# kehanxuuu/vspg-pbrt-v4

Measured on AMD Instinct MI355X. Metric: Mpaths/sec on 1920x1080 homogeneous fog; relMSE vs CPU ref at equal spp, higher is better.
Workload: dtype f32; 1 GPU; fog-box 1920x1080, guidedvolpathvspg vspguiding=true (primary-ray VSP; App. F options), 1 spp per step per GPU, independent sampler seed 0, maxdepth 5

## Files before the change

vspg-pbrt-v4_amd/csrc/vspg_capi.hip:

```cpp
#include <hip/hip_runtime.h>
#include <dlfcn.h>

#include <cmath>
#include <cstdio>
#include <cstdlib>
#include <cstring>
#include <string>
#include <type_traits>
#include <vector>
#include <algorithm>

#include "vspg_path.h"
#include "vspg_wg_kernel.h"
#include "vspg_guided_wg.h"
#include "vspg_wg3.h"
#include "vspg_trace.h"
#include "vspg_wavefront.h"
#include "vspg_wf_launch.h"
#include "vspg_film_error.h"
#ifdef VSPG_SINGLE_TU
#include "vspg_wf_grid.hip"
#include "vspg_wf_nvdb.hip"
#include "vspg_wg3_exact.hip"
#endif
// ... 1494 lines not shown
    float *le_scale = nullptr;
    float *temperature = nullptr;
    float *majorant = nullptr;
    DTri *tris = nullptr;
    DBvh4Node *bvh = nullptr;
    float *wf_pool = nullptr;
    float4 *wave_samples[2] = {nullptr, nullptr};
    int ws_cur = 0;
    bool ws_parked = false;
    PixelWindow ws_win = {0, 0, 0, 0};
    hipStream_t ws_stream = nullptr;
    hipEvent_t ws_event = nullptr;
    unsigned int *carry_img[2] = {nullptr, nullptr};
    int carry_cur = 0;
    bool carry_pending = false;
    Wg3Launch carry_shape = {};
    int carry_arith = 0;
    unsigned long long carry_resumes = 0;
    unsigned int *wf_lists = nullptr;
    hipStream_t wf_stream2 = nullptr;
    hipEvent_t wf_ev_vertex = nullptr, wf_ev_shadow = nullptr;
    WfIter *wf_iters = nullptr;
    size_t wf_items = 0;
    int num_cus = 0;
    int vsp_ready = 0;
    bool vsp_loaded = false;
    int wave_counter = 0, buffer_wave = 0;
    size_t npix = 0;
    float4 *fe_ref = nullptr;
    bool fe_ref_set = false;
// ... 1388 lines not shown
static bool wg2_defer_enabled() {
    const char *e = getenv("VSPG_WG2_DEFER");
    return !(e && e[0] == '0');
}
static int order_after_parking(VspgRenderer *r, hipStream_t s) {
    if (r->ws_parked && r->ws_event && s != r->ws_stream) HIPCHK(hipStreamWaitEvent(s, r->ws_event, 0));
    return 0;
}
static bool wg3_carry_enabled() {
    const char *e = getenv("VSPG_WG3_CARRY");
    return !(e && e[0] == '0') && wg2_defer_enabled();
}
static int wg3_launch_any(int arith, const Wg3Launch &L) {
    return arith == VSPG_ARITH_FAST_WEIGHTS ? vspg_arith1_wg3(&L) : arith == VSPG_ARITH_FAST ? vspg_arith2_wg3(&L) : wg3_launch_exact(L);
}
static int drain_carried_paths(VspgRenderer *r, hipStream_t s) {
    if (!r->carry_pending) return 0;
    if (const int rc = order_after_parking(r, s)) return rc;
    Wg3Launch L = r->carry_shape;
    L.vsp_ready = r->vsp_ready;
    L.first_sample = -1;
    L.work_head = r->work_head8 + (r->head8_parity & 1u) * (unsigned)(kWg3HeadSetBytes / 4);
    L.ws_prev = nullptr;
    L.ws_out = r->wave_samples[r->ws_cur ^ 1];
    L.stream = s;
    L.carry = 1;
    L.resume = r->carry_img[r->carry_cur ^ 1];
    L.suspend = nullptr;
    const int lrc = wg3_launch_any(r->carry_arith, L);
    if (lrc != 0) return fail(VSPG_EHIP, std::string("k_render_wave_wg3_carry (drain): ") + hipGetErrorName((hipError_t)lrc));
    r->carry_pending = false;
    r->ws_stream = s;
    if (r->ws_event) HIPCHK(hipEventRecord(r->ws_event, s));
    return 0;
}
static int flush_parked_samples(VspgRenderer *r, hipStream_t s) {
    if (const int rc = drain_carried_paths(r, s)) return rc;
    if (!r->ws_parked) return 0;
    if (const int rc = order_after_parking(r, s)) return rc;
    const size_t n_win = (size_t)(r->ws_win.x1 - r->ws_win.x0) * (size_t)(r->ws_win.y1 - r->ws_win.y0);
    hipLaunchKernelGGL(k_film_resolve, dim3((unsigned)((n_win + kBlock - 1) / kBlock)), dim3(kBlock), 0, s, r->cfg.xres, r->ws_win,
                       r->wave_samples[r->ws_cur ^ 1], r->film, r->isg_stats);
    HIPCHK(hipGetLastError());
    r->ws_parked = false;
    return 0;
}
static const char *kernel_name_exact(VspgRenderer *r);
const char *vspg_renderer_kernel_name(VspgRenderer *r) {
    if (!r) return "";
    if (r->arith == VSPG_ARITH_EXACT) return kernel_name_exact(r);
    r->kernel_name_buf = std::string(r->arith == VSPG_ARITH_FAST_WEIGHTS ? "fastw::" : "fast::") + kernel_name_exact(r);
    return r->kernel_name_buf.c_str();
// ... 89 lines not shown
    const int sc = r->cfg.shard_count, si = r->cfg.shard_index;
    int first = wave_start;
    if (sc > 1) first += ((si - wave_start % sc) % sc + sc) % sc;
    if (first >= wave_end) return 0;
    const int n_samples = (wave_end - 1 - first) / sc + 1;
    const PcgJump jump = pcg_jump((unsigned long long)first * 65536ull);
    const bool grid = r->scene.medium.type == VSPG_MEDIUM_GRID;
    const bool nvdb = r->scene.medium.type == VSPG_MEDIUM_NANOVDB;
    const bool guided = wants_guiding(r->prm);
    if (guided && !r->field_set) return fail(VSPG_ESCOPE, "guiding enabled but the renderer holds no guiding field");
    const bool defer = !uses_wf_pipeline(r) && uses_wg2(r) && n_samples == 1 && wg2_defer_enabled();
    const bool same_win = r->ws_win.x0 == x0 && r->ws_win.y0 == y0 && r->ws_win.x1 == x1 && r->ws_win.y1 == y1;
    if (!defer || !same_win) { const int rc = flush_parked_samples(r, (hipStream_t)stream); if (rc) return rc; }
    const bool carry = defer && uses_wg3(r) && !r->hscene.tr_calc && wg3_carry_enabled();
    if (r->carry_pending && !carry) { const int rc = drain_carried_paths(r, (hipStream_t)stream); if (rc) return rc; }
    if (uses_wf_pipeline(r)) {
#ifdef VSPG_WF_DEBUG
        auto checksum = [&](const void *dptr, size_t bytes) -> unsigned long long {
            if (!dptr || !bytes) return 0ull;
            std::vector<unsigned char> h(bytes);
            (void)hipDeviceSynchronize();
            (void)hipMemcpy(h.data(), dptr, bytes, hipMemcpyDeviceToHost);
            unsigned long long x = 1469598103934665603ull;
            for (size_t i = 0; i < bytes; ++i) { x ^= h[i]; x *= 1099511628211ull; }
            return x;
        };
        const size_t nb = (size_t)r->hscene.bnx * r->hscene.bny * r->hscene.bnz;
        const void *bufs[6] = {r->tris, r->bvh, r->brick_index, r->octets, r->dscene, r->majorant};
        const size_t sizes[6] = {(size_t)r->hscene.n_tris * sizeof(DTri), (size_t)r->hscene.n_bvh_nodes * sizeof(DBvh4Node), nb * 4, r->n_bricks * 512 * 32,
                                 sizeof(DScene), (size_t)16 * 16 * 16 * 4};
// ... 50 lines not shown
        long long wblocks = (long long)r->num_cus * (wwaves * 4 / (wblock / 64));
        const long long wmax = (items + kWgChunk - 1) / kWgChunk;
        if (wblocks > wmax) wblocks = wmax;
        const int single = n_samples == 1 ? 1 : 0;
        const long long n_tiles_all = (long long)tilesX * tilesY;
        const bool sched2 = uses_wg2(r);
        if (sched2) {
            for (int k = 0; k < 2; ++k)
                if (!r->wave_samples[k]) HIPCHK(hipMalloc(&r->wave_samples[k], r->npix * sizeof(float4)));
            const int wg3_grey = r->medium_grey ? (r->surfaces_grey ? 2 : 1) : 0, wg3_null_zero = r->medium_grey && r->surfaces_grey && r->null_zero ? 1 : 0;
            if (carry && wblocks > n_tiles_all) wblocks = n_tiles_all;
            if (r->carry_pending) {
                const Wg3Launch &P = r->carry_shape;
                const bool same_shape = carry && P.grey == wg3_grey && P.null_zero == wg3_null_zero && P.blocks == (unsigned)wblocks && P.windowed == (whole ? 0 : 1) &&
                                        r->carry_arith == r->arith && P.first_sample != first && P.dscene == r->dscene;
                if (!same_shape) { const int rc = drain_carried_paths(r, (hipStream_t)stream); if (rc) return rc; }
            }
            float4 *const ws_out = r->wave_samples[r->ws_cur];
            const float4 *const ws_prev = defer && r->ws_parked ? r->wave_samples[r->ws_cur ^ 1] : nullptr;
            if (ws_prev) { const int rc = order_after_parking(r, (hipStream_t)stream); if (rc) return rc; }
            const long long n_tiles = n_tiles_all;
            if (wblocks > n_tiles) wblocks = n_tiles;
            const int tail64 = [] { const char *e = getenv("VSPG_WG2_TAIL"); const int v = e ? atoi(e) : 64; return v < 0 ? 0 : (v > 64 ? 64 : v); }();
            const unsigned static_tiles = (unsigned)((n_tiles * (64 - tail64) / 64) / wblocks * wblocks);
#define VSPG_LAUNCH_WG2(M, G, NPOOL, BLK, WV)                                                                                         \
    hipLaunchKernelGGL((k_render_wave_wg2<M, G, NPOOL, BLK, WV>), dim3((unsigned)wblocks), dim3(BLK), 0, (hipStream_t)stream, r->dscene, \
                       r->film, r->isg_stats, r->vsp, r->vsp_ready, wave_end, first, single, jump, tiles_magic, static_tiles, work_head, ws_prev, ws_out, r->counters, targs, win)
            if (uses_wg3(r)) {
                {
                    static_assert(kWgBlockHomog == VSPG_WG_BLOCK && kWgWavesHomog == VSPG_WG_WAVES, "wg3_launch_unguided's launch shape");
                    unsigned int *const head8 = r->work_head8 + (r->head8_parity & 1u) * (unsigned)(kWg3HeadSetBytes / 4);
// ... 189 lines not shown
        }
        while (std::pow(2.0, (double)r->buffer_wave) <= (double)r->wave_counter) r->buffer_wave++;
    }
    return 0;
}
int vspg_post_process_wave(VspgRenderer *r, void *stream) { return vspg_post_process_step(r, 1, nullptr, stream); }
int vspg_renderer_set_exchange(VspgRenderer *r, VspgExchangeFn fn, void *user) {
    if (!r) return fail(VSPG_EINVAL, "null renderer");
    r->exchange = fn;
    r->exchange_user = user;
    return 0;
}

int vspg_flush(VspgRenderer *r, void *stream) {
    if (!r) return fail(VSPG_EINVAL, "null renderer");
    if (!r->ws_parked) return 0;
    HIPCHK(hipSetDevice(r->cfg.device));
    return flush_parked_samples(r, (hipStream_t)stream);
}
long long vspg_debug_carry_resumes(VspgRenderer *r) { return r ? (long long)r->carry_resumes : -1; }
int vspg_film_device_ptr(VspgRenderer *r, float **dev_ptr, size_t *n_floats) {
    if (!r || !dev_ptr || !n_floats) return fail(VSPG_EINVAL, "null argument");
    if (r->ws_parked) {
        HIPCHK(hipSetDevice(r->cfg.device));
        const hipStream_t s = r->ws_stream;
        if (const int rc = flush_parked_samples(r, s)) return rc;
        HIPCHK(hipStreamSynchronize(s));
    }
    *dev_ptr = reinterpret_cast<float *>(r->film);
    *n_floats = r->npix * 4;
    return 0;
}
int vspg_film_read(VspgRenderer *r, float *host, void *stream) {
    if (!r || !host) return fail(VSPG_EINVAL, "null argument");
    HIPCHK(hipSetDevice(r->cfg.device));
    if (const int rc = flush_parked_samples(r, (hipStream_t)stream)) return rc;
    HIPCHK(hipMemcpyAsync(host, r->film, r->npix * sizeof(float4), hipMemcpyDeviceToHost, (hipStream_t)stream));
    HIPCHK(hipStreamSynchronize((hipStream_t)stream));
// ... 115 lines not shown
    HIPCHK(hipStreamSynchronize(s));
    return 0;
}
int vspg_vsp_buffer_load(VspgRenderer *r, const float *host, void *stream) {
    if (!r || !host) return fail(VSPG_EINVAL, "null argument");
    HIPCHK(hipSetDevice(r->cfg.device));
    if (const int rc = flush_parked_samples(r, (hipStream_t)stream)) return rc;
    HIPCHK(hipMemcpyAsync(r->vsp, host, r->npix * sizeof(float), hipMemcpyHostToDevice, (hipStream_t)stream));
    HIPCHK(hipStreamSynchronize((hipStream_t)stream));
    r->vsp_ready = 1;
    r->vsp_loaded = true;
    return 0;
}
int vspg_isg_stats_device_ptr(VspgRenderer *r, float **dev_ptr, size_t *n_floats) {
    if (!r || !dev_ptr || !n_floats) return fail(VSPG_EINVAL, "null argument");
    if (r->ws_parked) {
        HIPCHK(hipSetDevice(r->cfg.device));
        const hipStream_t s = r->ws_stream;
        if (const int rc = flush_parked_samples(r, s)) return rc;
        HIPCHK(hipStreamSynchronize(s));
    }
    *dev_ptr = r->isg_stats;
    *n_floats = r->npix * VSPG_ISG_STATS;
    return 0;
}
int vspg_get_counters(VspgRenderer *r, VspgCounters *out, void *stream) {
    if (!r || !out) return fail(VSPG_EINVAL, "null argument");
    HIPCHK(hipSetDevice(r->cfg.device));
    if (const int rc = drain_carried_paths(r, (hipStream_t)stream)) return rc;
    unsigned long long h[kNumCounters];
    HIPCHK(hipMemcpyAsync(h, r->counters, sizeof h, hipMemcpyDeviceToHost, (hipStream_t)stream));
// ... 404 lines not shown
```

vspg-pbrt-v4_amd/csrc/vspg_wg3.h:

```cpp
#pragma once
#include <type_traits>

#include "vspg_guided_wg.h"
#include "vspg_path.h"
#include "vspg_wg_kernel.h"

VSPG_NS_BEGIN

enum { Q_VV = 0, Q_VS = 1, Q_A = 2, Q_F = 3, Q_COUNT = 4 };
enum { QC_RES = 0, QC_COM = 1, QC_HEAD = 2, QC_STRIDE = 4 };
enum { W3_BUSY_S = Q_COUNT * QC_STRIDE, W3_BUSY_V, W3_EXH, W3_LIVE, W3_COUNT };
enum { W3_OLD = Q_VV * QC_STRIDE + 3, W3_SUSP_LO = Q_VS * QC_STRIDE + 3, W3_SUSP_HI = Q_A * QC_STRIDE + 3 };
constexpr unsigned kCarryDrainBit = 0x80000000u;
enum { W3_NONE = 0, W3_VERTEX = 1, W3_SEGMENT = 2, W3_FRESH = 3, W3_EXIT = 4 };
constexpr unsigned kRestartBit = 0x8000u;

VDEV float isg_code(const IsgSample &isg) {
    if (!isg.valid) return 0.f;
    const float q = isg.vsp_used >= 0.f ? isg.vsp_used : 0.5f;
    return isg.surface_event ? -q : q;
}
__device__ __forceinline__ void resolve_sample(float4 s, float4 *film_px, float *isg_px) {
    const Spec L = Spec{s.x, s.y, s.z};
    film_add_sample_rmw(film_px, L);
    IsgSample isg;
    isg.valid = s.w != 0.f;
    isg.surface_event = s.w < 0.f;
    isg.vsp_used = __builtin_fabsf(s.w);
// ... 5 lines not shown
    return v;
}
__device__ __forceinline__ int w3_lane() {
    int l = (int)(threadIdx.x & 63u);
    asm volatile("" : "+v"(l));
    return l;
}
constexpr float kCarrySentinel = 2.f;
__device__ __forceinline__ bool carry_sentinel(float w) { return w > 1.f; }
template <class LY, int NP> constexpr int kWg3ImagePool = LY::COUNT * NP;
template <class LY, int NP> constexpr int kWg3ImageWords = LY::COUNT * NP + Q_COUNT * NP / 2;
template <class LY, int NP> constexpr int kWg3ImageStride = kWg3ImageWords<LY, NP> + 32;
static_assert(W3_COUNT <= 32, "the image's queue words");

constexpr int kWg3Heads = 8, kWg3HeadSetBytes = kWg3Heads * 128;
__device__ __forceinline__ void reset_sibling_head(unsigned int *work_head) {
    if (blockIdx.x == 0 && threadIdx.x == 0) *reinterpret_cast<unsigned int *>(reinterpret_cast<uintptr_t>(work_head) ^ 4u) = 0u;
}

typedef unsigned int w3_u32x4 __attribute__((ext_vector_type(4)));
typedef const volatile __attribute__((address_space(3))) w3_u32x4 *w3_lds_v4;
template <int NP>
VDEV void ring_push_all(int dq, unsigned entry, unsigned short (*ring)[NP], unsigned int *s_w) {
    const int lane = w3_lane();
    const unsigned long long m0 = __ballot(dq == 0), m1 = __ballot(dq == 1), m2 = __ballot(dq == 2), m3 = __ballot(dq == 3);
    const unsigned n0 = (unsigned)__popcll(m0), n1 = (unsigned)__popcll(m1), n2 = (unsigned)__popcll(m2), n3 = (unsigned)__popcll(m3);
    const unsigned myn = lane == 0 ? n0 : lane == 1 ? n1 : lane == 2 ? n2 : n3;
    unsigned base = 0;
    if (lane < Q_COUNT && myn > 0u) base = atomicAdd(s_w + lane * QC_STRIDE + QC_RES, myn);
    const unsigned b0 = (unsigned)__builtin_amdgcn_readlane((int)base, 0), b1 = (unsigned)__builtin_amdgcn_readlane((int)base, 1);
// ... 14 lines not shown
#define VSPG_WG3_NP_CAP 768
#endif
#ifndef VSPG_WG3_LDS_BUDGET
#define VSPG_WG3_LDS_BUDGET 81920
#endif
#ifndef VSPG_WG3_OTHER
#define VSPG_WG3_OTHER 5200
#endif
template <class LY>
constexpr int wg3_pool_paths(int other_bytes) {
    const int n = (VSPG_WG3_LDS_BUDGET - other_bytes) / (LY::COUNT * 4 + Q_COUNT * 2) / 32 * 32;
    return n < VSPG_WG3_NP_CAP ? n : VSPG_WG3_NP_CAP;
}

#ifdef VSPG_W3_TIMELINE
enum { W3T_BEGIN = 0, W3T_FULL, W3T_EXH, W3T_EXIT, W3T_SUMS, W3T_WORDS = W3T_SUMS + 27, W3T_MAX_BLOCKS = 2048 };
__device__ unsigned long long g_w3_timeline[W3T_MAX_BLOCKS][8][32];
struct W3Timeline {
    unsigned long long *rec, t0;
    unsigned phase;
    __device__ __forceinline__ bool mine() const { return (threadIdx.x & 63u) == 0u && blockIdx.x < (unsigned)W3T_MAX_BLOCKS; }
    __device__ __forceinline__ W3Timeline() : rec(&g_w3_timeline[blockIdx.x % W3T_MAX_BLOCKS][(threadIdx.x >> 6) & 7u][0]), t0(0), phase(0) { stamp(W3T_BEGIN); }
    __device__ __forceinline__ void stamp(int i) { const unsigned long long t = __builtin_amdgcn_s_memrealtime(); if (mine()) rec[i] = t; }
    __device__ __forceinline__ void enter(unsigned p, int i) { if (phase < p) { phase = p; stamp(i); } }
    __device__ __forceinline__ void chunk_begin() { t0 = __builtin_amdgcn_s_memrealtime(); }
    __device__ __forceinline__ void chunk_end(unsigned kind, unsigned lanes) {
        const unsigned long long t1 = __builtin_amdgcn_s_memrealtime();
        if (mine()) {
            unsigned long long *r = rec + W3T_SUMS + (phase * 3u + kind) * 3u;
            atomicAdd(r, 1ull); atomicAdd(r + 1, (unsigned long long)lanes); atomicAdd(r + 2, t1 - t0);
        }
    }
};
#define VSPG_W3T(x) x
#else
#define VSPG_W3T(x)
#endif

template <class Medium, bool GUIDED, int NP, int kWgBlock, int kWgWavesPerSimd, bool TRAIN, bool WINDOW, bool CARRY = false>
__device__ __forceinline__ void wg3_render(
    const DScene *__restrict__ Sp, float4 *__restrict__ film, float *__restrict__ isg_stats, const float *__restrict__ vsp_buf,
    int vsp_ready, int wave_end, int first_sample, int single_sample, PcgJump jump, unsigned int tiles_magic,
    unsigned int *__restrict__ work_head, const float4 *__restrict__ prev_samples,
    float4 *__restrict__ wave_samples, unsigned long long *__restrict__ counters, TrainArgs train, const PixelWindow win,
    const unsigned int *__restrict__ resume = nullptr, unsigned int *__restrict__ suspend = nullptr) {
    static_assert(!CARRY || (!TRAIN && !GUIDED), "CARRY serves the unguided one-sample launches");
    vsp_ready = w3_at_use(vsp_ready), wave_end = w3_at_use(wave_end), first_sample = w3_at_use(first_sample);
    single_sample = w3_at_use(single_sample);
    const DScene &S = *Sp;
    const int W = S.xres, H = S.yres;
    const int tilesX = WINDOW ? win_tiles_x(win) : (W + 7) >> 3, tilesY = WINDOW ? win_tiles_y(win) : (H + 7) >> 3;
    const unsigned n_tiles = CARRY && w3_at_use(suspend) == nullptr ? 0u : (unsigned)(tilesX * tilesY);
    const auto in_launch = [&](int px, int py) {
        if constexpr (WINDOW) return win_has(win, px, py);
        else return px < W && py < H;
    };
    const int lane = threadIdx.x & 63;
    const int sample_step = S.shard_count > 1 ? S.shard_count : 1;
    if (blockIdx.x == 0 && threadIdx.x < (unsigned)kWg3Heads)
        reinterpret_cast<unsigned int *>(reinterpret_cast<uintptr_t>(work_head) ^ (uintptr_t)kWg3HeadSetBytes)[threadIdx.x * 32u] = 0u;
    unsigned wseg = blockIdx.x % (unsigned)kWg3Heads, wtried = 0u;

    constexpr bool FULL = !Medium::kSimpleScene;
    static_assert(!FULL || !GUIDED, "the workgroup kernel's guided vertex (vspg_guided_wg.h) is built for rectangle scenes");
    static_assert(NP < (int)kRestartBit, "a ring entry is the slot plus the restart bit");
    using LY = PoolLayout<GUIDED, Medium::kGrey, TRAIN, FULL>;
    constexpr int NF = LY::COUNT;
    static_assert(!TRAIN || GUIDED, "segment recording belongs to the guided instantiations");
    static_assert(Medium::kSingleSegment, "k_render_wave_wg3 serves homogeneous media (grid media: the wavefront pipeline)");
    __shared__ float s_pool[NF * NP];
    __shared__ unsigned short s_ring[Q_COUNT][NP];
    __shared__ __attribute__((aligned(16))) unsigned int s_w[W3_COUNT];
    const Pool P{s_pool, NP};
    const Medium medium = MediumMaker<Medium>::make(S, nullptr);
    float *glds = nullptr;
    if constexpr (GUIDED && kKdLdsNodes > 0) {
        __shared__ VspgKdNode s_kd[2][kKdLdsNodes > 0 ? kKdLdsNodes : 1];
        for (int f = 0; f < 2; ++f) {
            const int nl = S.field[f].n_nodes < kKdLdsNodes ? S.field[f].n_nodes : kKdLdsNodes;
            for (int i = threadIdx.x; i < nl; i += kWgBlock) s_kd[f][i] = S.field[f].nodes[i];
        }
        glds = reinterpret_cast<float *>(&s_kd[0][0]);
    }
    __shared__ unsigned int s_counters[CNT_COUNT];
    struct LaneCounters : PathCounters { uint32_t paths; VDEV void path() { paths++; } };
    using Rec = typename std::conditional<TRAIN, PathRecorder, NullRecorder>::type;
// ... 7 lines not shown
            const unsigned tcol = WINDOW ? (px >> 3) - (unsigned)win_tile_x0(win) : px >> 3, trow = WINDOW ? (py >> 3) - (unsigned)win_tile_y0(win) : py >> 3;
            const unsigned item = (trow * (unsigned)tilesX + tcol) * 64u + ((py & 7u) << 3) + (px & 7u);
            pc.rec.base = train.segbuf + item;
            pc.rec.stride = (int)train.n_items;
            pc.rec.max_seg = train_rec_capacity(S.prm.maxdepth);
            return item;
        } else {
            (void)pxy;
            return 0u;
        }
    };

    stage_scene_lds(S);
    if (threadIdx.x < CNT_COUNT) s_counters[threadIdx.x] = 0;
    constexpr int kImgPool = kWg3ImagePool<LY, NP>, kImgWords = kWg3ImageWords<LY, NP>, kImgStride = kWg3ImageStride<LY, NP>;
    bool resumed = false;
    if constexpr (CARRY) {
        const unsigned int *const img = resume + (size_t)blockIdx.x * kImgStride;
        resumed = resume != nullptr && img[kImgWords + W3_LIVE] != 0u;
        if (resumed) {
            unsigned int *const pool32 = reinterpret_cast<unsigned int *>(s_pool);
#pragma unroll 8
            for (int i = threadIdx.x; i < kImgPool; i += kWgBlock) pool32[i] = img[i];
            unsigned short *const ring16 = &s_ring[0][0];
#pragma unroll 3
            for (int i = threadIdx.x; i < Q_COUNT * NP / 2; i += kWgBlock) {
                const unsigned v = img[kImgPool + i];
                ring16[2 * i] = (unsigned short)(v & 0xffffu);
                ring16[2 * i + 1] = (unsigned short)(v >> 16);
            }
            if (threadIdx.x < W3_COUNT) s_w[threadIdx.x] = img[kImgWords + threadIdx.x];
            __syncthreads();
            if (threadIdx.x < Q_COUNT) {
                const unsigned h = s_w[threadIdx.x * QC_STRIDE + QC_HEAD], n = s_w[threadIdx.x * QC_STRIDE + QC_COM] - h, h2 = h % (unsigned)NP;
                s_w[threadIdx.x * QC_STRIDE + QC_HEAD] = h2;
                s_w[threadIdx.x * QC_STRIDE + QC_RES] = h2 + n;
                s_w[threadIdx.x * QC_STRIDE + QC_COM] = h2 + n;
            }
            if (threadIdx.x == 0) {
                s_w[W3_OLD] = s_w[W3_LIVE];
                s_w[W3_EXH] = 0u;
                s_w[W3_BUSY_S] = 0u;
                s_w[W3_BUSY_V] = 0u;
            }
        }
    }
    if (!resumed) {
        if (threadIdx.x < W3_COUNT) s_w[threadIdx.x] = 0;
        for (int i = threadIdx.x; i < NP; i += kWgBlock) s_ring[Q_F][i] = (unsigned short)i;
        __syncthreads();
        if (threadIdx.x == 0) {
            s_w[Q_F * QC_STRIDE + QC_RES] = NP; s_w[Q_F * QC_STRIDE + QC_COM] = NP;
        }
    }
    if constexpr (CARRY) {
        __syncthreads();
        if (threadIdx.x == 0) {
            if (suspend == nullptr) { s_w[W3_EXH] = 1u; s_w[W3_OLD] |= kCarryDrainBit; }
            s_w[W3_SUSP_LO] = (unsigned)reinterpret_cast<uintptr_t>(suspend);
            s_w[W3_SUSP_HI] = (unsigned)(reinterpret_cast<uintptr_t>(suspend) >> 32);
        }
    }
    __syncthreads();

    auto emit = [&](int pxy, Spec Lraw, const IsgSample &isg, bool old) {
        const Spec L = finish_radiance(Lraw);
        const size_t pidx = (size_t)((unsigned)pxy >> 16) * W + (pxy & 0xffff);
        if (CARRY && old && w3_at_use(first_sample) >= 0) {
            resolve_sample(make_float4(L.r, L.g, L.b, isg_code(isg)), film + pidx, isg_stats + pidx * VSPG_ISG_STATS);
        } else if (w3_at_use(single_sample)) {
            wave_samples[pidx] = make_float4(L.r, L.g, L.b, isg_code(isg));
        } else {
            film_add_sample(film + pidx, L);
            isg_add_sample_atomic(isg_stats + pidx * VSPG_ISG_STATS, L, isg);
        }
    };

    VSPG_PROF(PS_WG_TOTAL);
    VSPG_PROF_ACC(prof_decide, PS_WG_R);
    VSPG_PROF_ACC(prof_idle, PS_WG_BAR_A);
    unsigned idle_polls = 0;
    VSPG_W3T(W3Timeline tl);
    while (true) {
        VSPG_PROF_ACC_BEGIN(prof_decide);
        VSPG_PROF_ACC_BEGIN(prof_idle);
        unsigned kind = W3_NONE, pos0 = 0, n0 = 0, pos1 = 0, n1 = 0, q0 = Q_VV, tile = 0;
        unsigned fresh_entry = 0;
        {
            const auto U = [](unsigned v) { return (unsigned)__builtin_amdgcn_readfirstlane((int)v); };
            const w3_lds_v4 qw = (w3_lds_v4)(s_w);
            const w3_u32x4 wVV = qw[Q_VV], wVS = qw[Q_VS], wA = qw[Q_A], wF = qw[Q_F], wM = qw[Q_COUNT];
            const unsigned hVV = U(wVV.z), hVS = U(wVS.z), hA = U(wA.z), hF = U(wF.z);
            const unsigned busyS = U(wM.x), busyV = U(wM.y), live = U(wM.w);
            const unsigned old_word = CARRY ? U(wVV.w) : 1u;
            const bool exh = U(wM.z) != 0u;
            VSPG_W3T(if (exh) tl.enter(2u, W3T_EXH));
            const auto avail = [&](w3_u32x4 q, unsigned head) {
                const unsigned r = U(q.x), c = U(q.y);
                const int a = (int)(c - head);
                return r == c && a > 0 ? a : 0;
            };
            const int aVV = avail(wVV, hVV), aVS = avail(wVS, hVS), aA = avail(wA, hA), aF = exh ? 0 : avail(wF, hF);
            const auto claim = [&](unsigned q, unsigned head, unsigned n) {
                unsigned old = head + 1u;
                if (w3_lane() == 0) old = atomicCAS(s_w + q * QC_STRIDE + QC_HEAD, head, head + n);
                return U(old) == head;
            };
            const auto bump = [&](int w, int d) { if (w3_lane() == 0) atomicAdd(s_w + w, (unsigned)d); };
            const auto claim_vertex = [&](int a_first, unsigned h_first, unsigned q_first, int a_second, unsigned h_second, unsigned q_second) {
                bump(W3_BUSY_V, 1);
// ... 13 lines not shown
                else bump(W3_BUSY_S, -1);
            };
            const int aV = aVV + aVS;
            if (CARRY && exh && old_word == 0u) kind = W3_EXIT;
            else if (aVV >= 64) claim_vertex(aVV, hVV, Q_VV, 0, hVS, Q_VS);
            else if (aVS >= 64) claim_vertex(aVS, hVS, Q_VS, 0, hVV, Q_VV);
            else if (aA >= 64) claim_segment();
            else if (aF >= 64) {
                bump(W3_BUSY_S, 1);
                bump(W3_LIVE, 64);
                if (claim(Q_F, hF, 64u)) {
                    kind = W3_FRESH; pos0 = hF; n0 = 64u;
                    __builtin_amdgcn_fence(__ATOMIC_ACQUIRE, "workgroup");
                    fresh_entry = s_ring[Q_F][(hF + (unsigned)lane) % (unsigned)NP];
                    tile = n_tiles;
                    while (wtried < (unsigned)kWg3Heads) {
                        unsigned c = 0xffffffffu;
                        if (w3_lane() == 0 && __hip_atomic_load(work_head + wseg * 32u, __ATOMIC_RELAXED, __HIP_MEMORY_SCOPE_AGENT) * (unsigned)kWg3Heads + wseg < n_tiles)
                            c = atomicAdd(work_head + wseg * 32u, 1u);
                        c = U(c);
                        if (c != 0xffffffffu && c * (unsigned)kWg3Heads + wseg < n_tiles) {
                            tile = c * (unsigned)kWg3Heads + wseg;
                            break;
                        }
                        wseg = (wseg + 1u) % (unsigned)kWg3Heads;
                        ++wtried;
                    }
                } else {
                    bump(W3_LIVE, -64);
                    bump(W3_BUSY_S, -1);
                }
            } else if (aV >= 64 || (aV > 0 && busyS == 0u)) {
                if (aVV >= aVS) claim_vertex(aVV, hVV, Q_VV, aVS, hVS, Q_VS);
                else claim_vertex(aVS, hVS, Q_VS, aVV, hVV, Q_VV);
            } else if (aA > 0 && busyV == 0u) {
                claim_segment();
            } else if (exh && live == 0u) {
                kind = W3_EXIT;
            }
        }
        if (kind == W3_EXIT) break;
        if (kind == W3_NONE) {
            if (idle_polls < 2u) __builtin_amdgcn_s_sleep(2);
            else __builtin_amdgcn_s_sleep(VSPG_WG3_IDLE_SLEEP);
            VSPG_PROF_ACC_END(prof_idle);
            if (++idle_polls > (1u << 23)) break;
            continue;
        }
        VSPG_PROF_ACC_END(prof_decide);
        idle_polls = 0;
        VSPG_W3T(if (kind == W3_VERTEX && n0 + n1 == 64u) tl.enter(1u, W3T_FULL); tl.chunk_begin());
        __builtin_amdgcn_fence(__ATOMIC_ACQUIRE, "workgroup");

        if (kind == W3_VERTEX) {
            VSPG_PROF(PS_WG_B);
            bool cont = false, restart = false, freed = false, old_done = false;
            int slot = 0;
            if ((unsigned)lane < n0 + n1) {
                slot = (unsigned)lane < n0 ? s_ring[q0][(pos0 + (unsigned)lane) % (unsigned)NP]
                                           : s_ring[q0 ^ 1u][(pos1 + ((unsigned)lane - n0)) % (unsigned)NP];
// ... 152 lines not shown
    VSPG_W3T(tl.stamp(W3T_EXIT));
    if constexpr (!GUIDED) {
        atomicAdd(&s_counters[CNT_PATHS], pc.paths); atomicAdd(&s_counters[CNT_SEGMENTS], pc.segments);
        atomicAdd(&s_counters[CNT_VOLUME_SCATTERS], pc.volume_scatters); atomicAdd(&s_counters[CNT_SURFACE_HITS], pc.surface_hits);
        atomicAdd(&s_counters[CNT_DENSITY_QUERIES], pc.density_queries); atomicAdd(&s_counters[CNT_SHADOW_RAYS], pc.shadow_rays);
        atomicAdd(&s_counters[CNT_SHADOW_QUERIES], pc.shadow_queries);
    }
    __syncthreads();
    if (threadIdx.x < CNT_COUNT) atomicAdd(&counters[threadIdx.x], (unsigned long long)s_counters[threadIdx.x]);
    if constexpr (CARRY) {
        unsigned int *const susp = reinterpret_cast<unsigned int *>((uintptr_t)s_w[W3_SUSP_LO] | ((uintptr_t)s_w[W3_SUSP_HI] << 32));
        if (susp != nullptr) {
            unsigned int *const img = susp + (size_t)blockIdx.x * kImgStride;
            if (threadIdx.x < W3_COUNT) img[kImgWords + threadIdx.x] = s_w[threadIdx.x];
            if (s_w[W3_LIVE] != 0u) {
                const unsigned int *const pool32 = reinterpret_cast<const unsigned int *>(s_pool);
                for (int i = threadIdx.x; i < kImgPool; i += kWgBlock) img[i] = pool32[i];
                const unsigned short *const ring16 = &s_ring[0][0];
                for (int i = threadIdx.x; i < Q_COUNT * NP / 2; i += kWgBlock) img[kImgPool + i] = (unsigned)ring16[2 * i] | ((unsigned)ring16[2 * i + 1] << 16);
                for (int q = 0; q < Q_F; ++q) {
                    const unsigned h = s_w[q * QC_STRIDE + QC_HEAD], n = s_w[q * QC_STRIDE + QC_COM] - h;
                    for (unsigned i = threadIdx.x; i < n && i < (unsigned)NP; i += kWgBlock) {
                        const int pxy = P.i(LY::PIXEL, (int)(s_ring[q][(h + i) % (unsigned)NP] & (kRestartBit - 1u)) % NP);
                        const unsigned px = (unsigned)pxy & 0xffffu, py = (unsigned)pxy >> 16;
                        if (in_launch((int)px, (int)py)) wave_samples[(size_t)py * W + px].w = kCarrySentinel;
                    }
                }
            }
        }
    }
}

template <class Medium, bool GUIDED, int NP, int kWgBlock, int kWgWavesPerSimd, bool TRAIN = false>
__global__ __launch_bounds__(kWgBlock, kWgWavesPerSimd) void k_render_wave_wg3(
    const DScene *__restrict__ Sp, float4 *__restrict__ film, float *__restrict__ isg_stats, const float *__restrict__ vsp_buf,
    int vsp_ready, int wave_end, int first_sample, int single_sample, PcgJump jump, unsigned int tiles_magic,
    unsigned int *__restrict__ work_head, const float4 *__restrict__ prev_samples,
    float4 *__restrict__ wave_samples, unsigned long long *__restrict__ counters, TrainArgs train = TrainArgs{nullptr, nullptr, nullptr, nullptr, 0, 0}) {
    wg3_render<Medium, GUIDED, NP, kWgBlock, kWgWavesPerSimd, TRAIN, false>(Sp, film, isg_stats, vsp_buf, vsp_ready, wave_end, first_sample, single_sample, jump,
                                                                            tiles_magic, work_head, prev_samples, wave_samples, counters, train, PixelWindow{0, 0, 0, 0});
}
template <class Medium, bool GUIDED, int NP, int kWgBlock, int kWgWavesPerSimd, bool TRAIN = false>
__global__ __launch_bounds__(kWgBlock, kWgWavesPerSimd) void k_render_wave_wg3_window(
    const DScene *__restrict__ Sp, float4 *__restrict__ film, float *__restrict__ isg_stats, const float *__restrict__ vsp_buf,
    int vsp_ready, int wave_end, int first_sample, int single_sample, PcgJump jump, unsigned int tiles_magic,
// ... 82 lines not shown
```

vspg-pbrt-v4_amd/csrc/vspg_wg3_exact.hip:

```cpp
#include <hip/hip_runtime.h>

#include "vspg_wg3.h"

VSPG_NS_BEGIN
int wg3_launch_exact(const Wg3Launch &L) { return wg3_launch_unguided(L); }
VSPG_NS_END

#ifdef VSPG_W3_TIMELINE
extern "C" int vspg_w3_timeline_read(unsigned long long *out, int blocks) {
    using namespace vspg;
    if (blocks < 0 || blocks > (int)W3T_MAX_BLOCKS) return -1;
    const size_t bytes = (size_t)blocks * 8 * 32 * sizeof(unsigned long long);
    if (hipDeviceSynchronize() != hipSuccess) return -2;
    if (hipMemcpyFromSymbol(out, HIP_SYMBOL(g_w3_timeline), bytes) != hipSuccess) return -3;
    void *p = nullptr;
    if (hipGetSymbolAddress(&p, HIP_SYMBOL(g_w3_timeline)) != hipSuccess || hipMemset(p, 0, sizeof(g_w3_timeline)) != hipSuccess) return -4;
    return 0;
}
#endif
```

Measured before the change: 3628 Mpaths/s.

## Fuse carried-path drain with parked-sample resolve and vectorize suspend images

When flushing, the carried-path drain launch now also resolves the parked wave samples and claims fresh tiles (exact arithmetic only), so a separate film-resolve kernel is no longer needed. In the carry kernel, exhaustion is detected by polling the global work heads, and a 'thin' drain mode relaxes the vertex/segment batching thresholds so stragglers finish sooner. The suspend and resume copies of the LDS image now use 128-bit accesses instead of 32-bit and 16-bit ones. Timeline instrumentation is extended with poll and branch counters. The changes add state (drain_behind) and cross-stream ordering that must stay correct for film reads.

```diff
diff --git a/vspg-pbrt-v4_amd/csrc/vspg_capi.hip b/vspg-pbrt-v4_amd/csrc/vspg_capi.hip
--- a/vspg-pbrt-v4_amd/csrc/vspg_capi.hip
+++ b/vspg-pbrt-v4_amd/csrc/vspg_capi.hip
@@ -1532,6 +1532,7 @@
     unsigned int *carry_img[2] = {nullptr, nullptr};
     int carry_cur = 0;
     bool carry_pending = false;
+    bool drain_behind = false;
     Wg3Launch carry_shape = {};
     int carry_arith = 0;
     unsigned long long carry_resumes = 0;
@@ -2950,14 +2951,21 @@
 static int wg3_launch_any(int arith, const Wg3Launch &L) {
     return arith == VSPG_ARITH_FAST_WEIGHTS ? vspg_arith1_wg3(&L) : arith == VSPG_ARITH_FAST ? vspg_arith2_wg3(&L) : wg3_launch_exact(L);
 }
-static int drain_carried_paths(VspgRenderer *r, hipStream_t s) {
+static int drain_carried_paths(VspgRenderer *r, hipStream_t s, bool resolve = false) {
     if (!r->carry_pending) return 0;
     if (const int rc = order_after_parking(r, s)) return rc;
+    resolve = resolve && r->ws_parked && r->carry_arith == VSPG_ARITH_EXACT;
     Wg3Launch L = r->carry_shape;
     L.vsp_ready = r->vsp_ready;
-    L.first_sample = -1;
     L.work_head = r->work_head8 + (r->head8_parity & 1u) * (unsigned)(kWg3HeadSetBytes / 4);
-    L.ws_prev = nullptr;
+    if (resolve) {
+        L.first_sample = L.wave_end = kCarryDrainResolve;
+        r->head8_parity ^= 1u;
+        L.ws_prev = r->wave_samples[r->ws_cur ^ 1];
+    } else {
+        L.first_sample = kCarryDrainPark;
+        L.ws_prev = nullptr;
+    }
     L.ws_out = r->wave_samples[r->ws_cur ^ 1];
     L.stream = s;
     L.carry = 1;
@@ -2968,10 +2976,20 @@
     r->carry_pending = false;
     r->ws_stream = s;
     if (r->ws_event) HIPCHK(hipEventRecord(r->ws_event, s));
+    if (resolve) {
+        r->ws_parked = false;
+        r->drain_behind = true;
+    }
+    return 0;
+}
+static int order_after_drain(VspgRenderer *r, hipStream_t s) {
+    if (r->drain_behind && r->ws_event && s != r->ws_stream) HIPCHK(hipStreamWaitEvent(s, r->ws_event, 0));
+    r->drain_behind = false;
     return 0;
 }
 static int flush_parked_samples(VspgRenderer *r, hipStream_t s) {
-    if (const int rc = drain_carried_paths(r, s)) return rc;
+    if (const int rc = drain_carried_paths(r, s, true)) return rc;
+    if (const int rc = order_after_drain(r, s)) return rc;
     if (!r->ws_parked) return 0;
     if (const int rc = order_after_parking(r, s)) return rc;
     const size_t n_win = (size_t)(r->ws_win.x1 - r->ws_win.x0) * (size_t)(r->ws_win.y1 - r->ws_win.y0);
@@ -3091,6 +3109,7 @@
     if (!defer || !same_win) { const int rc = flush_parked_samples(r, (hipStream_t)stream); if (rc) return rc; }
     const bool carry = defer && uses_wg3(r) && !r->hscene.tr_calc && wg3_carry_enabled();
     if (r->carry_pending && !carry) { const int rc = drain_carried_paths(r, (hipStream_t)stream); if (rc) return rc; }
+    if (const int rc = order_after_drain(r, (hipStream_t)stream)) return rc;
     if (uses_wf_pipeline(r)) {
 #ifdef VSPG_WF_DEBUG
         auto checksum = [&](const void *dptr, size_t bytes) -> unsigned long long {
@@ -3171,7 +3190,10 @@
                 const Wg3Launch &P = r->carry_shape;
                 const bool same_shape = carry && P.grey == wg3_grey && P.null_zero == wg3_null_zero && P.blocks == (unsigned)wblocks && P.windowed == (whole ? 0 : 1) &&
                                         r->carry_arith == r->arith && P.first_sample != first && P.dscene == r->dscene;
-                if (!same_shape) { const int rc = drain_carried_paths(r, (hipStream_t)stream); if (rc) return rc; }
+                if (!same_shape) {
+                    if (const int rc = drain_carried_paths(r, (hipStream_t)stream)) return rc;
+                    if (const int rc = order_after_drain(r, (hipStream_t)stream)) return rc;
+                }
             }
             float4 *const ws_out = r->wave_samples[r->ws_cur];
             const float4 *const ws_prev = defer && r->ws_parked ? r->wave_samples[r->ws_cur ^ 1] : nullptr;
@@ -3391,14 +3413,14 @@
 
 int vspg_flush(VspgRenderer *r, void *stream) {
     if (!r) return fail(VSPG_EINVAL, "null renderer");
-    if (!r->ws_parked) return 0;
+    if (!r->ws_parked && !r->drain_behind) return 0;
     HIPCHK(hipSetDevice(r->cfg.device));
     return flush_parked_samples(r, (hipStream_t)stream);
 }
 long long vspg_debug_carry_resumes(VspgRenderer *r) { return r ? (long long)r->carry_resumes : -1; }
 int vspg_film_device_ptr(VspgRenderer *r, float **dev_ptr, size_t *n_floats) {
     if (!r || !dev_ptr || !n_floats) return fail(VSPG_EINVAL, "null argument");
-    if (r->ws_parked) {
+    if (r->ws_parked || r->drain_behind) {
         HIPCHK(hipSetDevice(r->cfg.device));
         const hipStream_t s = r->ws_stream;
         if (const int rc = flush_parked_samples(r, s)) return rc;
@@ -3544,7 +3566,7 @@
 }
 int vspg_isg_stats_device_ptr(VspgRenderer *r, float **dev_ptr, size_t *n_floats) {
     if (!r || !dev_ptr || !n_floats) return fail(VSPG_EINVAL, "null argument");
-    if (r->ws_parked) {
+    if (r->ws_parked || r->drain_behind) {
         HIPCHK(hipSetDevice(r->cfg.device));
         const hipStream_t s = r->ws_stream;
         if (const int rc = flush_parked_samples(r, s)) return rc;
diff --git a/vspg-pbrt-v4_amd/csrc/vspg_wg3.h b/vspg-pbrt-v4_amd/csrc/vspg_wg3.h
--- a/vspg-pbrt-v4_amd/csrc/vspg_wg3.h
+++ b/vspg-pbrt-v4_amd/csrc/vspg_wg3.h
@@ -10,8 +10,9 @@
 enum { Q_VV = 0, Q_VS = 1, Q_A = 2, Q_F = 3, Q_COUNT = 4 };
 enum { QC_RES = 0, QC_COM = 1, QC_HEAD = 2, QC_STRIDE = 4 };
 enum { W3_BUSY_S = Q_COUNT * QC_STRIDE, W3_BUSY_V, W3_EXH, W3_LIVE, W3_COUNT };
-enum { W3_OLD = Q_VV * QC_STRIDE + 3, W3_SUSP_LO = Q_VS * QC_STRIDE + 3, W3_SUSP_HI = Q_A * QC_STRIDE + 3 };
+enum { W3_OLD = Q_VV * QC_STRIDE + 3, W3_SUSP_LO = Q_VS * QC_STRIDE + 3, W3_SUSP_HI = Q_A * QC_STRIDE + 3, W3_NEAR = Q_F * QC_STRIDE + 3 };
 constexpr unsigned kCarryDrainBit = 0x80000000u;
+constexpr int kCarryDrainPark = -1, kCarryDrainResolve = -2;
 enum { W3_NONE = 0, W3_VERTEX = 1, W3_SEGMENT = 2, W3_FRESH = 3, W3_EXIT = 4 };
 constexpr unsigned kRestartBit = 0x8000u;
 
@@ -47,6 +48,7 @@
 static_assert(W3_COUNT <= 32, "the image's queue words");
 
 constexpr int kWg3Heads = 8, kWg3HeadSetBytes = kWg3Heads * 128;
+constexpr unsigned kWg3NearTiles = 1024u;
 __device__ __forceinline__ void reset_sibling_head(unsigned int *work_head) {
     if (blockIdx.x == 0 && threadIdx.x == 0) *reinterpret_cast<unsigned int *>(reinterpret_cast<uintptr_t>(work_head) ^ 4u) = 0u;
 }
@@ -91,10 +93,12 @@
 }
 
 #ifdef VSPG_W3_TIMELINE
-enum { W3T_BEGIN = 0, W3T_FULL, W3T_EXH, W3T_EXIT, W3T_SUMS, W3T_WORDS = W3T_SUMS + 27, W3T_MAX_BLOCKS = 2048 };
-__device__ unsigned long long g_w3_timeline[W3T_MAX_BLOCKS][8][32];
+enum { W3T_BEGIN = 0, W3T_FULL, W3T_EXH, W3T_EXIT, W3T_SUMS, W3T_ENTRY = W3T_SUMS + 27, W3T_END, W3T_POLLS, W3T_POLL_TICKS, W3T_BRANCH,
+       W3T_WORDS = 48, W3T_MAX_BLOCKS = 2048 };
+static_assert(W3T_BRANCH + 6 <= W3T_WORDS, "a wavefront's record");
+__device__ unsigned long long g_w3_timeline[W3T_MAX_BLOCKS][8][W3T_WORDS];
 struct W3Timeline {
-    unsigned long long *rec, t0;
+    unsigned long long *rec, t0, tp;
     unsigned phase;
     __device__ __forceinline__ bool mine() const { return (threadIdx.x & 63u) == 0u && blockIdx.x < (unsigned)W3T_MAX_BLOCKS; }
     __device__ __forceinline__ W3Timeline() : rec(&g_w3_timeline[blockIdx.x % W3T_MAX_BLOCKS][(threadIdx.x >> 6) & 7u][0]), t0(0), phase(0) { stamp(W3T_BEGIN); }
@@ -106,7 +110,13 @@
         if (mine()) {
             unsigned long long *r = rec + W3T_SUMS + (phase * 3u + kind) * 3u;
             atomicAdd(r, 1ull); atomicAdd(r + 1, (unsigned long long)lanes); atomicAdd(r + 2, t1 - t0);
-        }
+            atomicAdd(rec + W3T_BRANCH + kind * 2u + (lanes < 64u ? 1u : 0u), 1ull);
+        }
+    }
+    __device__ __forceinline__ void poll_begin() { tp = __builtin_amdgcn_s_memrealtime(); }
+    __device__ __forceinline__ void poll_end() {
+        const unsigned long long t1 = __builtin_amdgcn_s_memrealtime();
+        if (mine()) { atomicAdd(rec + W3T_POLLS, 1ull); atomicAdd(rec + W3T_POLL_TICKS, t1 - tp); }
     }
 };
 #define VSPG_W3T(x) x
@@ -122,12 +132,13 @@
     float4 *__restrict__ wave_samples, unsigned long long *__restrict__ counters, TrainArgs train, const PixelWindow win,
     const unsigned int *__restrict__ resume = nullptr, unsigned int *__restrict__ suspend = nullptr) {
     static_assert(!CARRY || (!TRAIN && !GUIDED), "CARRY serves the unguided one-sample launches");
+    VSPG_W3T(const unsigned long long w3t_entry = __builtin_amdgcn_s_memrealtime());
     vsp_ready = w3_at_use(vsp_ready), wave_end = w3_at_use(wave_end), first_sample = w3_at_use(first_sample);
     single_sample = w3_at_use(single_sample);
     const DScene &S = *Sp;
     const int W = S.xres, H = S.yres;
     const int tilesX = WINDOW ? win_tiles_x(win) : (W + 7) >> 3, tilesY = WINDOW ? win_tiles_y(win) : (H + 7) >> 3;
-    const unsigned n_tiles = CARRY && w3_at_use(suspend) == nullptr ? 0u : (unsigned)(tilesX * tilesY);
+    const unsigned n_tiles = (unsigned)(tilesX * tilesY);
     const auto in_launch = [&](int px, int py) {
         if constexpr (WINDOW) return win_has(win, px, py);
         else return px < W && py < H;
@@ -145,8 +156,8 @@
     constexpr int NF = LY::COUNT;
     static_assert(!TRAIN || GUIDED, "segment recording belongs to the guided instantiations");
     static_assert(Medium::kSingleSegment, "k_render_wave_wg3 serves homogeneous media (grid media: the wavefront pipeline)");
-    __shared__ float s_pool[NF * NP];
-    __shared__ unsigned short s_ring[Q_COUNT][NP];
+    __shared__ __attribute__((aligned(16))) float s_pool[NF * NP];
+    __shared__ __attribute__((aligned(16))) unsigned short s_ring[Q_COUNT][NP];
     __shared__ __attribute__((aligned(16))) unsigned int s_w[W3_COUNT];
     const Pool P{s_pool, NP};
     const Medium medium = MediumMaker<Medium>::make(S, nullptr);
@@ -184,22 +195,27 @@
     stage_scene_lds(S);
     if (threadIdx.x < CNT_COUNT) s_counters[threadIdx.x] = 0;
     constexpr int kImgPool = kWg3ImagePool<LY, NP>, kImgWords = kWg3ImageWords<LY, NP>, kImgStride = kWg3ImageStride<LY, NP>;
+    constexpr int kImgPool4 = kImgPool / 4, kImgRing4 = Q_COUNT * NP / 8, kImgRounds = (kImgPool4 + kWgBlock - 1) / kWgBlock;
+    static_assert(NP % 32 == 0 && kImgPool % 4 == 0 && kImgStride % 4 == 0 && kImgRing4 <= kWgBlock, "the image copies' 128-bit accesses");
     bool resumed = false;
     if constexpr (CARRY) {
         const unsigned int *const img = resume + (size_t)blockIdx.x * kImgStride;
         resumed = resume != nullptr && img[kImgWords + W3_LIVE] != 0u;
         if (resumed) {
-            unsigned int *const pool32 = reinterpret_cast<unsigned int *>(s_pool);
-#pragma unroll 8
-            for (int i = threadIdx.x; i < kImgPool; i += kWgBlock) pool32[i] = img[i];
-            unsigned short *const ring16 = &s_ring[0][0];
-#pragma unroll 3
-            for (int i = threadIdx.x; i < Q_COUNT * NP / 2; i += kWgBlock) {
-                const unsigned v = img[kImgPool + i];
-                ring16[2 * i] = (unsigned short)(v & 0xffffu);
-                ring16[2 * i + 1] = (unsigned short)(v >> 16);
-            }
-            if (threadIdx.x < W3_COUNT) s_w[threadIdx.x] = img[kImgWords + threadIdx.x];
+            const w3_u32x4 *const img4 = reinterpret_cast<const w3_u32x4 *>(img);
+            w3_u32x4 *const pool4 = reinterpret_cast<w3_u32x4 *>(s_pool), *const ring4 = reinterpret_cast<w3_u32x4 *>(&s_ring[0][0]);
+            w3_u32x4 v[kImgRounds], vr;
+            unsigned vw;
+#pragma unroll
+            for (int k = 0; k < kImgRounds; ++k)
+                if ((k + 1) * kWgBlock <= kImgPool4 || (int)threadIdx.x + k * kWgBlock < kImgPool4) v[k] = img4[threadIdx.x + k * kWgBlock];
+            if ((int)threadIdx.x < kImgRing4) vr = img4[kImgPool4 + threadIdx.x];
+            if (threadIdx.x < W3_COUNT) vw = img[kImgWords + threadIdx.x];
+#pragma unroll
+            for (int k = 0; k < kImgRounds; ++k)
+                if ((k + 1) * kWgBlock <= kImgPool4 || (int)threadIdx.x + k * kWgBlock < kImgPool4) pool4[threadIdx.x + k * kWgBlock] = v[k];
+            if ((int)threadIdx.x < kImgRing4) ring4[threadIdx.x] = vr;
+            if (threadIdx.x < W3_COUNT) s_w[threadIdx.x] = vw;
             __syncthreads();
             if (threadIdx.x < Q_COUNT) {
                 const unsigned h = s_w[threadIdx.x * QC_STRIDE + QC_HEAD], n = s_w[threadIdx.x * QC_STRIDE + QC_COM] - h, h2 = h % (unsigned)NP;
@@ -210,6 +226,7 @@
             if (threadIdx.x == 0) {
                 s_w[W3_OLD] = s_w[W3_LIVE];
                 s_w[W3_EXH] = 0u;
+                s_w[W3_NEAR] = 0u;
                 s_w[W3_BUSY_S] = 0u;
                 s_w[W3_BUSY_V] = 0u;
             }
@@ -226,7 +243,10 @@
     if constexpr (CARRY) {
         __syncthreads();
         if (threadIdx.x == 0) {
-            if (suspend == nullptr) { s_w[W3_EXH] = 1u; s_w[W3_OLD] |= kCarryDrainBit; }
+            if (suspend == nullptr) {
+                s_w[W3_OLD] |= kCarryDrainBit;
+                if (first_sample == kCarryDrainPark) s_w[W3_EXH] = 1u;
+            }
             s_w[W3_SUSP_LO] = (unsigned)reinterpret_cast<uintptr_t>(suspend);
             s_w[W3_SUSP_HI] = (unsigned)(reinterpret_cast<uintptr_t>(suspend) >> 32);
         }
@@ -236,7 +256,7 @@
     auto emit = [&](int pxy, Spec Lraw, const IsgSample &isg, bool old) {
         const Spec L = finish_radiance(Lraw);
         const size_t pidx = (size_t)((unsigned)pxy >> 16) * W + (pxy & 0xffff);
-        if (CARRY && old && w3_at_use(first_sample) >= 0) {
+        if (CARRY && old && w3_at_use(first_sample) != kCarryDrainPark) {
             resolve_sample(make_float4(L.r, L.g, L.b, isg_code(isg)), film + pidx, isg_stats + pidx * VSPG_ISG_STATS);
         } else if (w3_at_use(single_sample)) {
             wave_samples[pidx] = make_float4(L.r, L.g, L.b, isg_code(isg));
@@ -250,8 +270,9 @@
     VSPG_PROF_ACC(prof_decide, PS_WG_R);
     VSPG_PROF_ACC(prof_idle, PS_WG_BAR_A);
     unsigned idle_polls = 0;
-    VSPG_W3T(W3Timeline tl);
+    VSPG_W3T(W3Timeline tl; if (tl.mine()) tl.rec[W3T_ENTRY] = w3t_entry);
     while (true) {
+        VSPG_W3T(tl.poll_begin());
         VSPG_PROF_ACC_BEGIN(prof_decide);
         VSPG_PROF_ACC_BEGIN(prof_idle);
         unsigned kind = W3_NONE, pos0 = 0, n0 = 0, pos1 = 0, n1 = 0, q0 = Q_VV, tile = 0;
@@ -263,7 +284,20 @@
             const unsigned hVV = U(wVV.z), hVS = U(wVS.z), hA = U(wA.z), hF = U(wF.z);
             const unsigned busyS = U(wM.x), busyV = U(wM.y), live = U(wM.w);
             const unsigned old_word = CARRY ? U(wVV.w) : 1u;
-            const bool exh = U(wM.z) != 0u;
+            const bool thin = CARRY && (old_word & kCarryDrainBit) != 0u;
+            bool exh = U(wM.z) != 0u;
+            if constexpr (CARRY) {
+                if (!exh && U(wF.w) != 0u) {
+                    const int l = w3_lane();
+                    bool left = false;
+                    if (l < kWg3Heads)
+                        left = __hip_atomic_load(work_head + l * 32, __ATOMIC_RELAXED, __HIP_MEMORY_SCOPE_AGENT) * (unsigned)kWg3Heads + (unsigned)l < n_tiles;
+                    if (__ballot(left) == 0ull) {
+                        exh = true;
+                        if (w3_lane() == 0) atomicExch(s_w + W3_EXH, 1u);
+                    }
+                }
+            }
             VSPG_W3T(if (exh) tl.enter(2u, W3T_EXH));
             const auto avail = [&](w3_u32x4 q, unsigned head) {
                 const unsigned r = U(q.x), c = U(q.y);
@@ -307,6 +341,27 @@
                     __builtin_amdgcn_fence(__ATOMIC_ACQUIRE, "workgroup");
                     fresh_entry = s_ring[Q_F][(hF + (unsigned)lane) % (unsigned)NP];
                     tile = n_tiles;
+                    if constexpr (CARRY) {
+                        while (wtried < (unsigned)kWg3Heads) {
+                            const int l = w3_lane();
+                            bool left = false;
+                            if (l < kWg3Heads)
+                                left = __hip_atomic_load(work_head + l * 32, __ATOMIC_RELAXED, __HIP_MEMORY_SCOPE_AGENT) * (unsigned)kWg3Heads + (unsigned)l < n_tiles;
+                            const unsigned m = (unsigned)__ballot(left);
+                            if (m == 0u) { wtried = (unsigned)kWg3Heads; break; }
+                            const unsigned rot = ((m >> wseg) | (m << ((unsigned)kWg3Heads - wseg))) & ((1u << kWg3Heads) - 1u);
+                            wseg = (wseg + (unsigned)__builtin_ctz(rot)) % (unsigned)kWg3Heads;
+                            unsigned c = 0xffffffffu;
+                            if (w3_lane() == 0) c = atomicAdd(work_head + wseg * 32u, 1u);
+                            c = U(c);
+                            if (c * (unsigned)kWg3Heads + wseg < n_tiles) {
+                                tile = c * (unsigned)kWg3Heads + wseg;
+                                break;
+                            }
+                            ++wtried;
+                        }
+                        if (tile + kWg3NearTiles >= n_tiles && w3_lane() == 0) s_w[W3_NEAR] = 1u;
+                    } else
                     while (wtried < (unsigned)kWg3Heads) {
                         unsigned c = 0xffffffffu;
                         if (w3_lane() == 0 && __hip_atomic_load(work_head + wseg * 32u, __ATOMIC_RELAXED, __HIP_MEMORY_SCOPE_AGENT) * (unsigned)kWg3Heads + wseg < n_tiles)
@@ -323,10 +378,10 @@
                     bump(W3_LIVE, -64);
                     bump(W3_BUSY_S, -1);
                 }
-            } else if (aV >= 64 || (aV > 0 && busyS == 0u)) {
+            } else if (aV >= 64 || (aV > 0 && (busyS == 0u || thin))) {
                 if (aVV >= aVS) claim_vertex(aVV, hVV, Q_VV, aVS, hVS, Q_VS);
                 else claim_vertex(aVS, hVS, Q_VS, aVV, hVV, Q_VV);
-            } else if (aA > 0 && busyV == 0u) {
+            } else if (aA > 0 && (busyV == 0u || thin)) {
                 claim_segment();
             } else if (exh && live == 0u) {
                 kind = W3_EXIT;
@@ -337,6 +392,7 @@
             if (idle_polls < 2u) __builtin_amdgcn_s_sleep(2);
             else __builtin_amdgcn_s_sleep(VSPG_WG3_IDLE_SLEEP);
             VSPG_PROF_ACC_END(prof_idle);
+            VSPG_W3T(tl.poll_end());
             if (++idle_polls > (1u << 23)) break;
             continue;
         }
@@ -519,10 +575,12 @@
             unsigned int *const img = susp + (size_t)blockIdx.x * kImgStride;
             if (threadIdx.x < W3_COUNT) img[kImgWords + threadIdx.x] = s_w[threadIdx.x];
             if (s_w[W3_LIVE] != 0u) {
-                const unsigned int *const pool32 = reinterpret_cast<const unsigned int *>(s_pool);
-                for (int i = threadIdx.x; i < kImgPool; i += kWgBlock) img[i] = pool32[i];
-                const unsigned short *const ring16 = &s_ring[0][0];
-                for (int i = threadIdx.x; i < Q_COUNT * NP / 2; i += kWgBlock) img[kImgPool + i] = (unsigned)ring16[2 * i] | ((unsigned)ring16[2 * i + 1] << 16);
+                w3_u32x4 *const img4 = reinterpret_cast<w3_u32x4 *>(img);
+                const w3_u32x4 *const pool4 = reinterpret_cast<const w3_u32x4 *>(s_pool), *const ring4 = reinterpret_cast<const w3_u32x4 *>(&s_ring[0][0]);
+#pragma unroll
+                for (int k = 0; k < kImgRounds; ++k)
+                    if ((k + 1) * kWgBlock <= kImgPool4 || (int)threadIdx.x + k * kWgBlock < kImgPool4) img4[threadIdx.x + k * kWgBlock] = pool4[threadIdx.x + k * kWgBlock];
+                if ((int)threadIdx.x < kImgRing4) img4[kImgPool4 + threadIdx.x] = ring4[threadIdx.x];
                 for (int q = 0; q < Q_F; ++q) {
                     const unsigned h = s_w[q * QC_STRIDE + QC_HEAD], n = s_w[q * QC_STRIDE + QC_COM] - h;
                     for (unsigned i = threadIdx.x; i < n && i < (unsigned)NP; i += kWgBlock) {
@@ -534,6 +592,7 @@
             }
         }
     }
+    VSPG_W3T(tl.stamp(W3T_END));
 }
 
 template <class Medium, bool GUIDED, int NP, int kWgBlock, int kWgWavesPerSimd, bool TRAIN = false>
diff --git a/vspg-pbrt-v4_amd/csrc/vspg_wg3_exact.hip b/vspg-pbrt-v4_amd/csrc/vspg_wg3_exact.hip
--- a/vspg-pbrt-v4_amd/csrc/vspg_wg3_exact.hip
+++ b/vspg-pbrt-v4_amd/csrc/vspg_wg3_exact.hip
@@ -10,7 +10,7 @@
 extern "C" int vspg_w3_timeline_read(unsigned long long *out, int blocks) {
     using namespace vspg;
     if (blocks < 0 || blocks > (int)W3T_MAX_BLOCKS) return -1;
-    const size_t bytes = (size_t)blocks * 8 * 32 * sizeof(unsigned long long);
+    const size_t bytes = (size_t)blocks * 8 * W3T_WORDS * sizeof(unsigned long long);
     if (hipDeviceSynchronize() != hipSuccess) return -2;
     if (hipMemcpyFromSymbol(out, HIP_SYMBOL(g_w3_timeline), bytes) != hipSuccess) return -3;
     void *p = nullptr;
```

Measured after the change: 2987 Mpaths/s. -17.7%, worse.
